# HaSai666/rec_pangu

Hardware: AMD Instinct MI355X
Metric: samples/sec DeepFM Criteo-shape bsz=65536/GPU (train step: fwd+bwd+dense Adam+zero_grad) (higher is better)
Workload: dtype f32

## Files before the change

rec_pangu_amd/csrc/mlp_tail.hip:

```cpp
#include "common.h"
#include "bfsplit.h"

#define MT_LD 72
#define MT_CT 68
#define MT_MAXL 3

struct TailFwdArgs {
    const float *W[MT_MAXL];
    const float *b[MT_MAXL];
    float *h[MT_MAXL];
    int64_t ldw[MT_MAXL];
};

__device__ __forceinline__ void mt_stage_w(const float *__restrict__ W, int64_t ldw, __bf16 (*Wt)[64][MT_LD]) {
    const int d = threadIdx.x >> 2, c = (threadIdx.x & 3) * 16;
    const float *src = W + (int64_t)d * ldw + c;
#pragma unroll
    for (int u = 0; u < 2; ++u) {
        const f32x4 v0 = *reinterpret_cast<const f32x4 *>(src + 8 * u), v1 = *reinterpret_cast<const f32x4 *>(src + 8 * u + 4);
        f32x8 v;
#pragma unroll
        for (int e = 0; e < 4; ++e) {
            v[e] = v0[e];
            v[4 + e] = v1[e];
        }
        bf16x8 pc[3];
        bf_split8<3>(v, pc);
#pragma unroll
        for (int q = 0; q < 3; ++q) *reinterpret_cast<bf16x8 *>(&Wt[q][d][c + 8 * u]) = pc[q];
    }
}

__device__ __forceinline__ void mt_stage_wt(const float *__restrict__ W, int64_t ldw, __bf16 (*Wt)[64][MT_LD]) {
    const int k = threadIdx.x >> 2, c = (threadIdx.x & 3) * 16;
    const float *src = W + (int64_t)k * ldw + c;
#pragma unroll
    for (int u = 0; u < 4; ++u) {
        const f32x4 v = *reinterpret_cast<const f32x4 *>(src + 4 * u);
#pragma unroll
        for (int e = 0; e < 4; ++e) {
            const float x = v[e];
            const __bf16 hi = (__bf16)x;
            const float r1 = x - (float)hi;
            const __bf16 mid = (__bf16)r1;
            const __bf16 lo = (__bf16)(r1 - (float)mid);
            const int n = c + 4 * u + e;
            Wt[0][n][k] = hi;
            Wt[1][n][k] = mid;
            Wt[2][n][k] = lo;
        }
    }
}

struct TailBce {
    const float *add[3];
    int n_add;
    const float *label;
    float p_eps;
    float *pred;
    float *partial;
};

template <int L, bool BCE>
__global__ __launch_bounds__(256, 2) void mlp_tail_fwd_kernel(const float *__restrict__ hin, int64_t ldin, TailFwdArgs a,
                                                              const float *__restrict__ wout, const float *__restrict__ bout,
                                                              float *__restrict__ logit, int64_t M, TailBce bc) {
    __shared__ __attribute__((aligned(16))) __bf16 Wt[3][64][MT_LD];
    __shared__ __attribute__((aligned(16))) float Ct[4][32][MT_CT];
    const int wv = threadIdx.x >> 6, l = threadIdx.x & 63, i = l & 31, h = l >> 5;
    const int64_t row = (int64_t)blockIdx.x * 128 + 32 * wv + i;
    const int64_t rowc = row < M ? row : M - 1;
    f32x8 av[4];
    {
        const float *src = hin + rowc * ldin + 8 * h;
#pragma unroll
        for (int ks = 0; ks < 4; ++ks) {
            const f32x4 v0 = *reinterpret_cast<const f32x4 *>(src + ks * 16), v1 = *reinterpret_cast<const f32x4 *>(src + ks * 16 + 4);
#pragma unroll
            for (int e = 0; e < 4; ++e) {
                av[ks][e] = v0[e];
                av[ks][4 + e] = v1[e];
            }
        }
    }
#pragma unroll
    for (int ly = 0; ly < L; ++ly) {
        if (ly > 0) __syncthreads();
        mt_stage_w(a.W[ly], a.ldw[ly], Wt);
        __syncthreads();
        f32x16 acc[2];
#pragma unroll
        for (int nt = 0; nt < 2; ++nt)
#pragma unroll
            for (int r = 0; r < 16; ++r) acc[nt][r] = 0.f;
#pragma unroll
        for (int ks = 0; ks < 4; ++ks) {
            bf16x8 af[3];
            bf_split8<3>(av[ks], af);
#pragma unroll
            for (int nt = 0; nt < 2; ++nt) {
                bf16x8 b[3];
#pragma unroll
                for (int q = 0; q < 3; ++q) b[q] = *reinterpret_cast<const bf16x8 *>(&Wt[q][nt * 32 + i][ks * 16 + 8 * h]);
#pragma unroll
                for (int pr = 0; pr < 6; ++pr)
                    acc[nt] = __builtin_amdgcn_mfma_f32_32x32x16_bf16(af[BfProd<6>::pa(pr)], b[BfProd<6>::pb(pr)], acc[nt], 0, 0, 0);
            }
        }
        float *hout = a.h[ly];
#pragma unroll
        for (int nt = 0; nt < 2; ++nt) {
            const int n = nt * 32 + i;
            const float bv = a.b[ly] != nullptr ? a.b[ly][n] : 0.f;
#pragma unroll
            for (int r = 0; r < 16; ++r) {
                const int rl = (r & 3) + 8 * (r >> 2) + 4 * h;
                const float v = fmaxf(acc[nt][r] + bv, 0.f);
                Ct[wv][rl][n] = v;
                const int64_t m = (int64_t)blockIdx.x * 128 + 32 * wv + rl;
                if (m < M) hout[m * 64 + n] = v;
            }
        }
        __syncthreads();
#pragma unroll
        for (int ks = 0; ks < 4; ++ks) {
            const f32x4 v0 = *reinterpret_cast<const f32x4 *>(&Ct[wv][i][ks * 16 + 8 * h]);
            const f32x4 v1 = *reinterpret_cast<const f32x4 *>(&Ct[wv][i][ks * 16 + 8 * h + 4]);
#pragma unroll
            for (int e = 0; e < 4; ++e) {
                av[ks][e] = v0[e];
                av[ks][4 + e] = v1[e];
            }
        }
    }
    float part = 0.f;
#pragma unroll
    for (int ks = 0; ks < 4; ++ks)
#pragma unroll
        for (int e = 0; e < 8; ++e) part = __builtin_fmaf(av[ks][e], wout[ks * 16 + 8 * h + e], part);
    part += __shfl_xor(part, 32, 64);
    const float lg = part + (bout != nullptr ? bout[0] : 0.f);
    if constexpr (!BCE) {
        if (h == 0 && row < M) logit[row] = lg;
    } else {
        __shared__ float lred[128];
        if (h == 0) {
            float term = 0.f;
            if (row < M) {
                float z = lg;
                if (bc.n_add > 0) {
                    z = bc.add[0][row];
                    for (int q = 1; q < bc.n_add; ++q) z += bc.add[q][row];
                    z += lg;
                }
                const float p = 1.f / (1.f + expf(-z));
                bc.pred[row] = p;
                const float pe = p + bc.p_eps, y = bc.label[row];
                const float lp = fmaxf(logf(pe), -100.f), l1p = fmaxf(log1pf(-pe), -100.f);
                term = -(y * lp + (1.f - y) * l1p);
            }
            lred[32 * wv + i] = term;
        }
        __syncthreads();
        if (threadIdx.x < 64) {
            float v = lred[threadIdx.x] + lred[threadIdx.x + 64];
#pragma unroll
            for (int o = 32; o >= 1; o >>= 1) v += __shfl_xor(v, o, 64);
            if (threadIdx.x == 0) bc.partial[blockIdx.x] = v;
        }
    }
}

extern "C" int rp_mlp_tail_fits(int n_hidden, int width, int64_t ldin) {
    return (n_hidden >= 1 && n_hidden <= MT_MAXL && width == 64 && ldin % 4 == 0) ? 1 : 0;
}

static int tail_fwd_launch(const float *hin, int64_t ldin, int n_hidden, const float *const *W_hidden, const int64_t *ldw,
                           const float *const *b_hidden, float *const *h_out, const float *w_out, const float *b_out,
                           float *logit, int64_t M, const TailBce *bce, rp_stream_t stream) {
    RP_REQUIRE(hin && W_hidden && ldw && b_hidden && h_out && w_out && (logit || bce), "mlp_tail_fwd: null pointer");
    if (!rp_mlp_tail_fits(n_hidden, 64, ldin) || !rp_aligned16(hin))
        return rp_fail(RP_ERR_UNSUPPORTED, "mlp_tail_fwd: 1..3 hidden layers of width 64, 16-byte aligned rows");
    if (M == 0) return RP_OK;
    TailFwdArgs a;
    for (int l = 0; l < MT_MAXL; ++l) {
        a.W[l] = nullptr;
        a.b[l] = nullptr;
        a.h[l] = nullptr;
        a.ldw[l] = 0;
    }
    for (int l = 0; l < n_hidden; ++l) {
        RP_REQUIRE(W_hidden[l] && h_out[l] && ldw[l] >= 64 && ldw[l] % 4 == 0 && rp_aligned16(W_hidden[l]),
                   "mlp_tail_fwd: layer %d invalid", l);
        a.W[l] = W_hidden[l];
        a.b[l] = b_hidden[l];
        a.h[l] = h_out[l];
        a.ldw[l] = ldw[l];
    }
    const dim3 grid((unsigned)rp_cdiv(M, 128));
    hipStream_t s = (hipStream_t)stream;
    TailBce bc{};
    if (bce != nullptr) bc = *bce;
#define TAIL_FWD(LL, BB) hipLaunchKernelGGL((mlp_tail_fwd_kernel<LL, BB>), grid, dim3(256), 0, s, hin, ldin, a, w_out, b_out, logit, M, bc)
    if (bce == nullptr) {
        if (n_hidden == 1) TAIL_FWD(1, false);
        else if (n_hidden == 2) TAIL_FWD(2, false);
        else TAIL_FWD(3, false);
    } else {
        if (n_hidden == 1) TAIL_FWD(1, true);
        else if (n_hidden == 2) TAIL_FWD(2, true);
        else TAIL_FWD(3, true);
    }
#undef TAIL_FWD
    RP_LAUNCH_CHECK("mlp_tail_fwd");
    return RP_OK;
}

extern "C" int rp_mlp_tail_fwd(const float *hin, int64_t ldin, int n_hidden, const float *const *W_hidden, const int64_t *ldw,
                               const float *const *b_hidden, float *const *h_out, const float *w_out, const float *b_out,
                               float *logit, int64_t M, rp_stream_t stream) {
    RP_REQUIRE(logit != nullptr, "mlp_tail_fwd: null pointer");
    return tail_fwd_launch(hin, ldin, n_hidden, W_hidden, ldw, b_hidden, h_out, w_out, b_out, logit, M, nullptr, stream);
}

extern "C" int rp_mlp_tail_loss_partials(int64_t M) { return (int)rp_cdiv(M > 0 ? M : 1, 128); }
// ... 7 lines not shown
    TailBce bc{};
    for (int q = 0; q < n_addends; ++q) {
        RP_REQUIRE(addends[q] != nullptr, "mlp_tail_fwd_bce: null addend %d", q);
        bc.add[q] = addends[q];
    }
    bc.n_add = n_addends;
    bc.label = label;
    bc.p_eps = p_eps;
    bc.pred = pred;
    bc.partial = partial;
    return tail_fwd_launch(hin, ldin, n_hidden, W_hidden, ldw, b_hidden, h_out, w_out, b_out, nullptr, M, &bc, stream);
}

struct TailBwdArgs {
    const float *W[MT_MAXL];
    const float *act[MT_MAXL + 1];
    int64_t ldw[MT_MAXL];
    int64_t ldact0;
};

struct TailDz {
    const float *pred, *label, *gloss;
    float p_eps, scale;
    float *dz_out;
};

template <int L>
__global__ __launch_bounds__(256, 2) void mlp_tail_bwd_kernel(const float *__restrict__ dz, TailBwdArgs a,
                                                              const float *__restrict__ wout, float *__restrict__ dhin,
                                                              int64_t lddh, float *__restrict__ P, int64_t M, int nwg, TailDz tz) {
    __shared__ __attribute__((aligned(16))) float T0[4][32][MT_CT];
    __shared__ __attribute__((aligned(16))) float T1[4][32][MT_CT];
    __shared__ float dzs[128];
    const int wv = threadIdx.x >> 6, l = threadIdx.x & 63, i = l & 31, h = l >> 5;
    const int64_t row0 = (int64_t)blockIdx.x * 128;
    const int64_t row = row0 + 32 * wv + i;
    const bool rok = row < M;
    const int64_t rowc = rok ? row : M - 1;
    const int mt = wv & 1, ntw = wv >> 1;
    float (*T0f)[MT_CT] = reinterpret_cast<float (*)[MT_CT]>(&T0[0][0][0]);
    float (*T1f)[MT_CT] = reinterpret_cast<float (*)[MT_CT]>(&T1[0][0][0]);
    float *Pg = P + (int64_t)blockIdx.x * ((int64_t)L * 64 * 64 + (int64_t)L * 64 + 64 + 1);
    float dzr = 0.f;
    if (tz.pred == nullptr) {
        dzr = rok ? dz[row] : 0.f;
    } else if (rok) {
        const float g = tz.gloss[0] * tz.scale;
        const float p = tz.pred[row], y = tz.label[row], pe = p + tz.p_eps;
        dzr = (pe - y) / fmaxf((1.f - pe) * pe, 1e-12f) * g;
        dzr *= p * (1.f - p);
        if (h == 0 && tz.dz_out != nullptr) tz.dz_out[row] = dzr;
    }
    if (h == 0) dzs[32 * wv + i] = dzr;
    f32x8 dp[4];
    {
        const float *src = a.act[L] + rowc * 64 + 8 * h;
#pragma unroll
        for (int ks = 0; ks < 4; ++ks) {
            const f32x4 v0 = *reinterpret_cast<const f32x4 *>(src + ks * 16), v1 = *reinterpret_cast<const f32x4 *>(src + ks * 16 + 4);
#pragma unroll
            for (int e = 0; e < 8; ++e) {
                const float av = e < 4 ? v0[e] : v1[e - 4];
                dp[ks][e] = av > 0.f ? dzr * wout[ks * 16 + 8 * h + e] : 0.f;
                T1[wv][i][ks * 16 + 8 * h + e] = rok ? dzr * av : 0.f;
            }
        }
    }
    __syncthreads();
    if (threadIdx.x < 64) {
        float s = 0.f;
        for (int r = 0; r < 128; ++r) s += T1f[r][threadIdx.x];
        Pg[(int64_t)L * 64 * 64 + (int64_t)L * 64 + threadIdx.x] = s;
    } else if (threadIdx.x == 64) {
        float s = 0.f;
        for (int r = 0; r < 128; ++r) s += dzs[r];
        Pg[(int64_t)L * 64 * 64 + (int64_t)L * 64 + 64] = s;
    }
#pragma unroll
    for (int ly = L; ly >= 1; --ly) {
        __syncthreads();
#pragma unroll
        for (int ks = 0; ks < 4; ++ks)
#pragma unroll
            for (int e = 0; e < 8; ++e) T0[wv][i][ks * 16 + 8 * h + e] = dp[ks][e];
        {
            const float *src = (ly - 1 == 0 ? a.act[0] + rowc * a.ldact0 : a.act[ly - 1] + rowc * 64) + 8 * h;
#pragma unroll
            for (int ks = 0; ks < 4; ++ks) {
                const f32x4 v0 = *reinterpret_cast<const f32x4 *>(src + ks * 16), v1 = *reinterpret_cast<const f32x4 *>(src + ks * 16 + 4);
                *reinterpret_cast<f32x4 *>(&T1[wv][i][ks * 16 + 8 * h]) = rok ? v0 : f32x4{0.f, 0.f, 0.f, 0.f};
                *reinterpret_cast<f32x4 *>(&T1[wv][i][ks * 16 + 8 * h + 4]) = rok ? v1 : f32x4{0.f, 0.f, 0.f, 0.f};
            }
        }
        bf16x8 wf[2][4][3];
        {
            const float *Wl = a.W[ly - 1];
            const int64_t ldw = a.ldw[ly - 1];
#pragma unroll
            for (int nt = 0; nt < 2; ++nt)
#pragma unroll
                for (int ks = 0; ks < 4; ++ks) {
                    f32x8 v;
#pragma unroll
                    for (int e = 0; e < 8; ++e) v[e] = Wl[(int64_t)(ks * 16 + 8 * h + e) * ldw + nt * 32 + i];
                    bf_split8<3>(v, wf[nt][ks]);
                }
        }
        __syncthreads();
        f32x16 wacc;
#pragma unroll
        for (int r = 0; r < 16; ++r) wacc[r] = 0.f;
        float bsum = 0.f;
#pragma unroll
        for (int ks = 0; ks < 8; ++ks) {
            f32x8 va, vb;
#pragma unroll
            for (int e = 0; e < 8; ++e) {
                va[e] = T0f[ks * 16 + 8 * h + e][mt * 32 + i];
                vb[e] = T1f[ks * 16 + 8 * h + e][ntw * 32 + i];
            }
            bsum += ((va[0] + va[1]) + (va[2] + va[3])) + ((va[4] + va[5]) + (va[6] + va[7]));
            bf16x8 pa_[3], pb_[3];
            bf_split8<3>(va, pa_);
            bf_split8<3>(vb, pb_);
#pragma unroll
            for (int pr = 0; pr < 6; ++pr)
                wacc = __builtin_amdgcn_mfma_f32_32x32x16_bf16(pa_[BfProd<6>::pa(pr)], pb_[BfProd<6>::pb(pr)], wacc, 0, 0, 0);
        }
        {
            float *Pw = Pg + (int64_t)(ly - 1) * 64 * 64;
#pragma unroll
            for (int r = 0; r < 16; ++r) Pw[(mt * 32 + (r & 3) + 8 * (r >> 2) + 4 * h) * 64 + ntw * 32 + i] = wacc[r];
            bsum += __shfl_xor(bsum, 32, 64);
            if (ntw == 0 && h == 0) Pg[(int64_t)L * 64 * 64 + (int64_t)(ly - 1) * 64 + mt * 32 + i] = bsum;
        }
        f32x16 acc[2];
#pragma unroll
        for (int nt = 0; nt < 2; ++nt)
#pragma unroll
            for (int r = 0; r < 16; ++r) acc[nt][r] = 0.f;
#pragma unroll
        for (int ks = 0; ks < 4; ++ks) {
            bf16x8 af[3];
            bf_split8<3>(dp[ks], af);
#pragma unroll
            for (int nt = 0; nt < 2; ++nt) {
#pragma unroll
                for (int pr = 0; pr < 6; ++pr)
                    acc[nt] = __builtin_amdgcn_mfma_f32_32x32x16_bf16(af[BfProd<6>::pa(pr)], wf[nt][ks][BfProd<6>::pb(pr)], acc[nt], 0, 0, 0);
            }
        }
        __syncthreads();
#pragma unroll
        for (int nt = 0; nt < 2; ++nt) {
            const int n = nt * 32 + i;
#pragma unroll
            for (int r = 0; r < 16; ++r) {
                const int rl = (r & 3) + 8 * (r >> 2) + 4 * h;
                const float v = T1[wv][rl][n] > 0.f ? acc[nt][r] : 0.f;
                if (ly - 1 == 0) {
                    const int64_t m = row0 + 32 * wv + rl;
                    if (m < M) dhin[m * lddh + n] = v;
                } else {
                    T0[wv][rl][n] = v;
                }
            }
        }
        if (ly - 1 > 0) {
            __syncthreads();
#pragma unroll
            for (int ks = 0; ks < 4; ++ks) {
                const f32x4 v0 = *reinterpret_cast<const f32x4 *>(&T0[wv][i][ks * 16 + 8 * h]);
                const f32x4 v1 = *reinterpret_cast<const f32x4 *>(&T0[wv][i][ks * 16 + 8 * h + 4]);
#pragma unroll
                for (int e = 0; e < 4; ++e) {
                    dp[ks][e] = v0[e];
                    dp[ks][4 + e] = v1[e];
                }
            }
        }
    }
}

__global__ __launch_bounds__(256) void mlp_tail_reduce_kernel(const float *__restrict__ P, int nwg, int64_t per, float *__restrict__ out) {
    __shared__ float red[16][17];
    const int c = threadIdx.x & 15, q = threadIdx.x >> 4;
    const int64_t e = (int64_t)blockIdx.x * 16 + c;
    float s = 0.f;
    if (e < per)
        for (int g = q; g < nwg; g += 16) s += P[(int64_t)g * per + e];
    red[q][c] = s;
    __syncthreads();
    if (q != 0 || e >= per) return;
#pragma unroll
    for (int j = 1; j < 16; ++j) s += red[j][c];
    out[e] = s;
}

extern "C" int rp_mlp_tail_bwd_workspace_bytes(int64_t M, int n_hidden, size_t *bytes) {
    RP_REQUIRE(bytes && M >= 0 && n_hidden >= 1 && n_hidden <= MT_MAXL, "mlp_tail_bwd_workspace_bytes: bad argument");
    const int64_t per = (int64_t)n_hidden * 64 * 64 + (int64_t)n_hidden * 64 + 64 + 1;
    *bytes = (size_t)(rp_cdiv(M > 0 ? M : 1, 128) * per) * sizeof(float) + 256;
// ... 81 lines not shown
```

rec_pangu_amd/csrc/embed_tiny.hip:

```cpp
#include "common.h"
#include "bfsplit.h"

#define ET_MAXF 16
#define ET_ROWS 224
#define ET_COLS 160
#define ET_LD 72
#define ET_CHUNK 64
#define ET_NOROW 254
#define ET_NOSMP 255

struct TinyTables {
    int n, total;
    int field[ET_MAXF];
    int base[ET_MAXF];
    int rows[ET_MAXF];
    int acc0[ET_MAXF];
};

__device__ __forceinline__ void tiny_split3(float v, __bf16 *p0, __bf16 *p1, __bf16 *p2) {
    uint32_t u = __float_as_uint(v);
    *reinterpret_cast<uint16_t *>(p0) = (uint16_t)(u >> 16);
    v -= __uint_as_float(u & 0xFFFF0000u);
    u = __float_as_uint(v);
    *reinterpret_cast<uint16_t *>(p1) = (uint16_t)(u >> 16);
    v -= __uint_as_float(u & 0xFFFF0000u);
    u = __float_as_uint(v);
    *reinterpret_cast<uint16_t *>(p2) = (uint16_t)(u >> 16);
}

__global__ __launch_bounds__(256, 2) void embed_grad_tiny_partial_kernel(
    const int32_t *__restrict__ keys, int64_t B, TinyTables tt, const float *__restrict__ dh, int64_t lddh,
    const float *__restrict__ sum_in, const float *__restrict__ gfm, int64_t per_blk, float *__restrict__ partial) {
    __shared__ __attribute__((aligned(16))) __bf16 Zt[3][ET_COLS][ET_LD];
    __shared__ __attribute__((aligned(8))) uint8_t rid[ET_MAXF][ET_CHUNK];
    __shared__ uint8_t rfld[ET_ROWS], rloc[ET_ROWS];
    const int t = threadIdx.x, wv = t >> 6, l = t & 63, i = l & 31, h = l >> 5;
    for (int m = t; m < ET_ROWS; m += 256) {
        int slot = 0, loc = ET_NOROW;
        for (int j = 0; j < tt.n; ++j)
            if (m >= tt.acc0[j] && m < tt.acc0[j] + tt.rows[j]) {
                slot = j;
                loc = m - tt.acc0[j];
            }
        rfld[m] = (uint8_t)slot;
        rloc[m] = (uint8_t)loc;
    }
    for (int e = t; e < 3 * (ET_COLS - 130) * ET_LD; e += 256) {
        const int p = e / ((ET_COLS - 130) * ET_LD), rest = e - p * ((ET_COLS - 130) * ET_LD);
        Zt[p][130 + rest / ET_LD][rest % ET_LD] = (__bf16)0.f;
    }
    f32x16 acc[5];
#pragma unroll
    for (int nt = 0; nt < 5; ++nt)
#pragma unroll
        for (int r = 0; r < 16; ++r) acc[nt][r] = 0.f;
    const int64_t s_begin = (int64_t)blockIdx.x * per_blk;
    const int64_t s_end = s_begin + per_blk < B ? s_begin + per_blk : B;
    __syncthreads();
    const int mt = 4 * (int)blockIdx.y + wv;
    const bool mok = mt < ET_ROWS / 32;
    const int fl0 = mok ? rfld[32 * mt + i] : 0, lc0 = mok ? rloc[32 * mt + i] : ET_NOROW;
    const int s = t >> 2, q = t & 3;
    f32x4 vd[4], vs[4];
    float g = 0.f, okf = 0.f;
    int rloc0 = ET_NOSMP, rloc1 = ET_NOSMP;
    auto fetch = [&](int64_t c0) {
        const int64_t b = c0 + s;
        const bool ok = b < s_end;
        const int64_t bc = ok ? b : s_end - 1;
        okf = ok ? 1.f : 0.f;
        g = (gfm != nullptr) ? gfm[bc] * okf : 0.f;
#pragma unroll
        for (int e = 0; e < 4; ++e) vd[e] = *reinterpret_cast<const f32x4 *>(dh + bc * lddh + 16 * q + 4 * e);
        if (sum_in != nullptr) {
#pragma unroll
            for (int e = 0; e < 4; ++e) vs[e] = *reinterpret_cast<const f32x4 *>(sum_in + bc * 64 + 16 * q + 4 * e);
        }
        rloc0 = rloc1 = ET_NOSMP;
        {
            const int idx = t, j = idx >> 6, ss = idx & 63;
            if (idx < tt.n * ET_CHUNK && c0 + ss < s_end) rloc0 = keys[(int64_t)tt.field[j] * B + c0 + ss] - tt.base[j];
        }
        {
            const int idx = t + 256, j = idx >> 6, ss = idx & 63;
            if (idx < tt.n * ET_CHUNK && c0 + ss < s_end) rloc1 = keys[(int64_t)tt.field[j] * B + c0 + ss] - tt.base[j];
        }
    };
    fetch(s_begin);
    for (int64_t c0 = s_begin; c0 < s_end; c0 += ET_CHUNK) {
        {
#pragma unroll
            for (int e = 0; e < 16; ++e) {
                const int col = 16 * q + e;
                tiny_split3(vd[e >> 2][e & 3] * okf, &Zt[0][col][s], &Zt[1][col][s], &Zt[2][col][s]);
                const float uval = (sum_in != nullptr) ? g * vs[e >> 2][e & 3] : 0.f;
                tiny_split3(uval, &Zt[0][64 + col][s], &Zt[1][64 + col][s], &Zt[2][64 + col][s]);
            }
            if (q == 0) tiny_split3(g, &Zt[0][128][s], &Zt[1][128][s], &Zt[2][128][s]);
            if (q == 1) tiny_split3(okf, &Zt[0][129][s], &Zt[1][129][s], &Zt[2][129][s]);
            if (t < tt.n * ET_CHUNK) rid[t >> 6][t & 63] = (uint8_t)rloc0;
            if (t + 256 < tt.n * ET_CHUNK) rid[(t + 256) >> 6][t & 63] = (uint8_t)rloc1;
            for (int idx = t + 512; idx < tt.n * ET_CHUNK; idx += 256) {
                const int j = idx >> 6, ss = idx & 63;
                int loc = ET_NOSMP;
                if (c0 + ss < s_end) loc = keys[(int64_t)tt.field[j] * B + c0 + ss] - tt.base[j];
                rid[j][ss] = (uint8_t)loc;
            }
        }
        if (c0 + ET_CHUNK < s_end) fetch(c0 + ET_CHUNK);
        __syncthreads();
#pragma unroll
        for (int ks = 0; ks < 4; ++ks) {
            const uint64_t r8 = *reinterpret_cast<const uint64_t *>(&rid[fl0][16 * ks + 8 * h]);
            u32x4 aw;
#pragma unroll
            for (int j = 0; j < 4; ++j) {
                const uint32_t e0 = (uint32_t)((r8 >> (16 * j)) & 0xFF), e1 = (uint32_t)((r8 >> (16 * j + 8)) & 0xFF);
                aw[j] = (e0 == (uint32_t)lc0 ? 0x00003F80u : 0u) | (e1 == (uint32_t)lc0 ? 0x3F800000u : 0u);
            }
            const bf16x8 a = __builtin_bit_cast(bf16x8, aw);
            if (mok) {
#pragma unroll
                for (int nt = 0; nt < 5; ++nt)
#pragma unroll
                    for (int p = 2; p >= 0; --p) {
                        const bf16x8 bq = *reinterpret_cast<const bf16x8 *>(&Zt[p][32 * nt + i][16 * ks + 8 * h]);
                        acc[nt] = __builtin_amdgcn_mfma_f32_32x32x16_bf16(a, bq, acc[nt], 0, 0, 0);
                    }
            }
        }
        __syncthreads();
    }
    float *P = partial + (int64_t)blockIdx.x * ET_ROWS * ET_COLS;
    if (mok) {
#pragma unroll
        for (int nt = 0; nt < 5; ++nt)
#pragma unroll
            for (int r = 0; r < 16; ++r)
                P[(int64_t)(32 * mt + (r & 3) + 8 * (r >> 2) + 4 * h) * ET_COLS + 32 * nt + i] = acc[nt][r];
    }
}

#define ET_FIN_PARTS 4
__global__ __launch_bounds__(ET_COLS * ET_FIN_PARTS) void embed_grad_tiny_finish_kernel(
    const float *__restrict__ partial, int nblk, TinyTables tt, const float *__restrict__ wt, int64_t ldwt,
    const float *__restrict__ arena, float *__restrict__ G, int accumulate, int has_fm, float *__restrict__ hs_out) {
    __shared__ float Sp[ET_FIN_PARTS][ET_COLS];
    __shared__ float S[ET_COLS];
    const int m = blockIdx.x, c = threadIdx.x % ET_COLS, part = threadIdx.x / ET_COLS;
    int slot = 0;
    for (int j = 0; j < tt.n; ++j)
        if (m >= tt.acc0[j] && m < tt.acc0[j] + tt.rows[j]) slot = j;
    const int64_t arow = (int64_t)tt.base[slot] + (m - tt.acc0[slot]);
    {
        const int per = (nblk + ET_FIN_PARTS - 1) / ET_FIN_PARTS;
        const int b0 = part * per, b1 = (b0 + per < nblk) ? b0 + per : nblk;
        float s = 0.f;
#pragma unroll 8
        for (int b = b0; b < b1; ++b) s += partial[((int64_t)b * ET_ROWS + m) * ET_COLS + c];
        Sp[part][c] = s;
    }
// ... 54 lines not shown
                                  int64_t ldwt, const float *gfm, const float *sum_in, const float *arena,
                                  float *grad_arena, int accumulate, float *dw, int64_t lddw, void *workspace,
                                  size_t workspace_bytes, rp_stream_t stream) {
    RP_REQUIRE(keys && tiny_field && tiny_base && tiny_rows && dh && wt && grad_arena && workspace, "embed_grad_tiny: null pointer");
    RP_REQUIRE(n_tiny >= 1 && n_tiny <= ET_MAXF, "embed_grad_tiny: %d tables (1..%d)", n_tiny, ET_MAXF);
    RP_REQUIRE(B >= 1 && B < INT32_MAX, "embed_grad_tiny: bad B");
    RP_REQUIRE(gfm == nullptr || arena != nullptr, "embed_grad_tiny: the FM term needs the arena");
    RP_REQUIRE(lddh % 4 == 0 && ldwt >= 64 && rp_aligned16(dh) && (sum_in == nullptr || rp_aligned16(sum_in)),
               "embed_grad_tiny: dh / sum_in rows must be 16-byte aligned");
    TinyTables tt;
    tt.n = n_tiny;
    int total = 0;
    for (int j = 0; j < ET_MAXF; ++j) {
        tt.field[j] = tt.base[j] = tt.rows[j] = tt.acc0[j] = 0;
        if (j >= n_tiny) continue;
        RP_REQUIRE(tiny_rows[j] >= 1 && tiny_rows[j] <= ET_NOROW, "embed_grad_tiny: table %d has %d rows (1..%d)", j, tiny_rows[j],
                   ET_NOROW);
        RP_REQUIRE(tiny_base[j] >= 0 && tiny_base[j] < INT32_MAX && tiny_field[j] >= 0, "embed_grad_tiny: bad table %d", j);
        tt.field[j] = tiny_field[j];
        tt.base[j] = (int)tiny_base[j];
        tt.rows[j] = tiny_rows[j];
        tt.acc0[j] = total;
        total += tiny_rows[j];
    }
    RP_REQUIRE(total <= ET_ROWS, "embed_grad_tiny: %d rows together (<= %d)", total, ET_ROWS);
    tt.total = total;
    const int64_t per = tiny_per_block(B);
    const int64_t nblk = rp_cdiv(B, per);
    size_t need = 0;
    rp_embed_grad_tiny_workspace_bytes(B, &need);
    RP_REQUIRE(workspace_bytes >= need, "embed_grad_tiny: workspace %zu < %zu bytes", workspace_bytes, need);
    float *partial = reinterpret_cast<float *>((reinterpret_cast<uintptr_t>(workspace) + 255) & ~(uintptr_t)255);
    hipStream_t s = (hipStream_t)stream;
    hipLaunchKernelGGL(embed_grad_tiny_partial_kernel, dim3((unsigned)nblk, 2), dim3(256), 0, s, keys, B, tt, dh, lddh, sum_in, gfm, per,
                       partial);
    RP_LAUNCH_CHECK("embed_grad_tiny (partial sums)");
    RP_REQUIRE(dw == nullptr || arena != nullptr, "embed_grad_tiny: the weight gradient needs the arena");
    float *hs = dw ? partial + (size_t)nblk * ET_ROWS * ET_COLS : nullptr;
    hipLaunchKernelGGL(embed_grad_tiny_finish_kernel, dim3((unsigned)total), dim3(ET_COLS * ET_FIN_PARTS), 0, s, partial, (int)nblk, tt, wt, ldwt, arena,
                       grad_arena, accumulate, gfm != nullptr ? 1 : 0, hs);
    RP_LAUNCH_CHECK("embed_grad_tiny (finish)");
    if (dw != nullptr) {
        for (int j = 0; j < n_tiny; ++j)
            RP_REQUIRE(lddw >= ((int64_t)tt.field[j] + 1) * 64, "embed_grad_tiny: dw rows shorter than field %d's columns", tt.field[j]);
        hipLaunchKernelGGL(embed_grad_tiny_dw_kernel, dim3((unsigned)n_tiny, 16), dim3(256), 0, s, hs, tt, arena, dw, lddw);
        RP_LAUNCH_CHECK("embed_grad_tiny (weight gradient)");
    }
    return RP_OK;
}
```

Measured before the change: 86.94 million.

## Prefetch weights and activations across layers in fused MLP tail kernels

The forward kernel now loads the next layer's weights into registers while the current layer computes. It writes hidden activations as coalesced 16-byte rows from the shared tile instead of scattered scalar stores, and it preloads biases, the output weight, labels and addends. Two block-wide barriers become wave-level syncs. The backward kernel prefetches the next layer's activations and transposed weights, stages W^T through shared memory (aliased onto T0) instead of uncoalesced per-lane global gathers, and vectorizes its tile writes. The cost is extra register pressure and an extra pair of barriers per backward layer.

After: 85.96 million. 0.989x the previous value.

```diff
diff --git a/profiles/microbench/mlp_tail.py b/profiles/microbench/mlp_tail.py
--- /dev/null
+++ b/profiles/microbench/mlp_tail.py
@@ -0,0 +1,77 @@
+import ctypes as C
+import json
+import sys
+import torch
+sys.path.insert(0, '.')
+from bench import HBM_COPY_GBS
+from rec_pangu_amd import hip
+
+args = [a for a in sys.argv[1:] if not a.startswith('--')]
+if '--lib' in sys.argv:
+    hip.LIB_PATH = sys.argv[sys.argv.index('--lib') + 1]
+    args.remove(hip.LIB_PATH)
+M = int(args[0]) if len(args) > 0 else 65536
+L = int(args[1]) if len(args) > 1 else 2
+reps = int(args[2]) if len(args) > 2 else 200
+lib = hip.lib()
+dev = 'cuda'
+g = torch.Generator(device=dev).manual_seed(0)
+rnd = lambda *s: torch.randn(*s, device=dev, generator=g)
+hin = rnd(M, 64).relu()
+Ws = [rnd(64, 64) / 8 for _ in range(L)]
+bs = [rnd(64) * 0.1 for _ in range(L)]
+w_out, b_out = rnd(1, 64) / 8, rnd(1)
+fm = rnd(M)
+label = (torch.rand(M, device=dev, generator=g) < 0.3).float()
+gloss = torch.tensor(1.0, device=dev)
+hs = [torch.empty(M, 64, device=dev) for _ in range(L)]
+pred = torch.empty(M, device=dev)
+n_part = lib.rp_mlp_tail_loss_partials(M)
+partial = torch.empty(n_part, device=dev)
+dhin = torch.empty(M, 64, device=dev)
+dz_out = torch.empty(M, device=dev)
+per = L * 4096 + L * 64 + 65
+grads = torch.empty(per, device=dev)
+nbytes = C.c_size_t(0)
+hip._check(lib.rp_mlp_tail_bwd_workspace_bytes(M, L, C.byref(nbytes)), "workspace")
+ws = torch.empty(nbytes.value, dtype=torch.uint8, device=dev)
+Wp, ldw = hip._ptr_array(Ws), hip._i64_array([64] * L)
+acts = hip._ptr_array([hin] + hs)
+
+
+def fwd():
+    hip._check(lib.rp_mlp_tail_fwd_bce(hin.data_ptr(), 64, L, Wp, ldw, hip._opt_ptr_array(bs), hip._ptr_array(hs), w_out.data_ptr(),
+                                       b_out.data_ptr(), hip._ptr_array([fm]), 1, label.data_ptr(), 0.0, pred.data_ptr(),
+                                       partial.data_ptr(), M, hip._stream()), "rp_mlp_tail_fwd_bce")
+
+
+def bwd():
+    hip._check(lib.rp_mlp_tail_bwd_bce(pred.data_ptr(), label.data_ptr(), gloss.data_ptr(), 0.0, 1.0, dz_out.data_ptr(), L, Wp, ldw,
+                                       acts, 64, w_out.data_ptr(), dhin.data_ptr(), 64, grads.data_ptr(), M, ws.data_ptr(),
+                                       nbytes.value, 1, hip._stream()), "rp_mlp_tail_bwd_bce")
+
+
+def time_us(fn):
+    for _ in range(20):
+        fn()
+    e0, e1 = torch.cuda.Event(enable_timing=True), torch.cuda.Event(enable_timing=True)
+    torch.cuda.synchronize()
+    e0.record()
+    for _ in range(reps):
+        fn()
+    e1.record()
+    torch.cuda.synchronize()
+    return e0.elapsed_time(e1) * 1e3 / reps
+
+
+nwg = (M + 127) // 128
+moved = {
+    "fwd": 4 * (M * 64 * (L + 1) + 3 * M + n_part) + 4 * L * 4160,
+    "bwd": 4 * (M * 64 * (L + 2) + 3 * M + nwg * per) + 4 * L * 4096,
+}
+for name, fn in (("fwd", fwd), ("bwd", bwd)):
+    us = time_us(fn)
+    gbs = moved[name] / us * 1e-3
+    print(json.dumps({"launch": f"mlp_tail_{name}_kernel<{L}>", "M": M, "lib": hip.LIB_PATH.split('/')[-2:], "alone_us": round(us, 2),
+                      "mbytes": round(moved[name] / 1e6, 2), "gb_per_s": round(gbs, 1),
+                      "frac_of_copy_ceiling": round(gbs / HBM_COPY_GBS, 3), "us_at_copy_ceiling": round(moved[name] / HBM_COPY_GBS * 1e-3, 2)}))
diff --git a/rec_pangu_amd/csrc/mlp_tail.hip b/rec_pangu_amd/csrc/mlp_tail.hip
--- a/rec_pangu_amd/csrc/mlp_tail.hip
+++ b/rec_pangu_amd/csrc/mlp_tail.hip
@@ -12,17 +12,23 @@
     int64_t ldw[MT_MAXL];
 };
 
-__device__ __forceinline__ void mt_stage_w(const float *__restrict__ W, int64_t ldw, __bf16 (*Wt)[64][MT_LD]) {
+
+__device__ __forceinline__ void mt_load_w(const float *__restrict__ W, int64_t ldw, f32x4 (&v)[4]) {
     const int d = threadIdx.x >> 2, c = (threadIdx.x & 3) * 16;
     const float *src = W + (int64_t)d * ldw + c;
 #pragma unroll
+    for (int u = 0; u < 4; ++u) v[u] = *reinterpret_cast<const f32x4 *>(src + 4 * u);
+}
+
+__device__ __forceinline__ void mt_store_w(const f32x4 (&r)[4], __bf16 (*Wt)[64][MT_LD]) {
+    const int d = threadIdx.x >> 2, c = (threadIdx.x & 3) * 16;
+#pragma unroll
     for (int u = 0; u < 2; ++u) {
-        const f32x4 v0 = *reinterpret_cast<const f32x4 *>(src + 8 * u), v1 = *reinterpret_cast<const f32x4 *>(src + 8 * u + 4);
         f32x8 v;
 #pragma unroll
         for (int e = 0; e < 4; ++e) {
-            v[e] = v0[e];
-            v[4 + e] = v1[e];
+            v[e] = r[2 * u][e];
+            v[4 + e] = r[2 * u + 1][e];
         }
         bf16x8 pc[3];
         bf_split8<3>(v, pc);
@@ -31,25 +37,31 @@
     }
 }
 
-__device__ __forceinline__ void mt_stage_wt(const float *__restrict__ W, int64_t ldw, __bf16 (*Wt)[64][MT_LD]) {
-    const int k = threadIdx.x >> 2, c = (threadIdx.x & 3) * 16;
-    const float *src = W + (int64_t)k * ldw + c;
-#pragma unroll
-    for (int u = 0; u < 4; ++u) {
-        const f32x4 v = *reinterpret_cast<const f32x4 *>(src + 4 * u);
-#pragma unroll
-        for (int e = 0; e < 4; ++e) {
-            const float x = v[e];
-            const __bf16 hi = (__bf16)x;
-            const float r1 = x - (float)hi;
-            const __bf16 mid = (__bf16)r1;
-            const __bf16 lo = (__bf16)(r1 - (float)mid);
-            const int n = c + 4 * u + e;
-            Wt[0][n][k] = hi;
-            Wt[1][n][k] = mid;
-            Wt[2][n][k] = lo;
-        }
-    }
+__device__ __forceinline__ void mt_load_wt(const float *__restrict__ W, int64_t ldw, float (&v)[16]) {
+    const int n = threadIdx.x & 63, kg = threadIdx.x >> 6;
+    const float *src = W + (int64_t)(16 * kg) * ldw + n;
+#pragma unroll
+    for (int e = 0; e < 16; ++e) v[e] = src[(int64_t)e * ldw];
+}
+
+__device__ __forceinline__ void mt_store_wt(const float (&r)[16], __bf16 (*Wt)[64][MT_LD]) {
+    const int n = threadIdx.x & 63, kg = threadIdx.x >> 6;
+#pragma unroll
+    for (int u = 0; u < 2; ++u) {
+        f32x8 v;
+#pragma unroll
+        for (int e = 0; e < 8; ++e) v[e] = r[8 * u + e];
+        bf16x8 pc[3];
+        bf_split8<3>(v, pc);
+#pragma unroll
+        for (int q = 0; q < 3; ++q) *reinterpret_cast<bf16x8 *>(&Wt[q][n][16 * kg + 8 * u]) = pc[q];
+    }
+}
+
+__device__ __forceinline__ void mt_wave_sync() {
+    __builtin_amdgcn_fence(__ATOMIC_RELEASE, "wavefront");
+    __builtin_amdgcn_wave_barrier();
+    __builtin_amdgcn_fence(__ATOMIC_ACQUIRE, "wavefront");
 }
 
 struct TailBce {
@@ -67,9 +79,12 @@
                                                               float *__restrict__ logit, int64_t M, TailBce bc) {
     __shared__ __attribute__((aligned(16))) __bf16 Wt[3][64][MT_LD];
     __shared__ __attribute__((aligned(16))) float Ct[4][32][MT_CT];
+    __shared__ __attribute__((aligned(16))) float wos[64];
     const int wv = threadIdx.x >> 6, l = threadIdx.x & 63, i = l & 31, h = l >> 5;
     const int64_t row = (int64_t)blockIdx.x * 128 + 32 * wv + i;
     const int64_t rowc = row < M ? row : M - 1;
+    f32x4 wr[4];
+    mt_load_w(a.W[0], a.ldw[0], wr);
     f32x8 av[4];
     {
         const float *src = hin + rowc * ldin + 8 * h;
@@ -83,10 +98,37 @@
             }
         }
     }
+    float bv[L][2];
+#pragma unroll
+    for (int ly = 0; ly < L; ++ly)
+#pragma unroll
+        for (int nt = 0; nt < 2; ++nt) bv[ly][nt] = a.b[ly] != nullptr ? a.b[ly][nt * 32 + i] : 0.f;
+    if (threadIdx.x < 64) wos[threadIdx.x] = wout[threadIdx.x];
+    const float bo = bout != nullptr ? bout[0] : 0.f;
+    float yl = 0.f, ad[3] = {0.f, 0.f, 0.f};
+    if constexpr (BCE) {
+        if (h == 0 && row < M) {
+            yl = bc.label[row];
+#pragma unroll
+            for (int q = 0; q < 3; ++q)
+                if (q < bc.n_add) ad[q] = bc.add[q][row];
+        }
+    }
+    auto store_rows = [&](float *hout) {
+        const int rs = l >> 4, cs = (l & 15) * 4;
+#pragma unroll
+        for (int j = 0; j < 8; ++j) {
+            const f32x4 v = *reinterpret_cast<const f32x4 *>(&Ct[wv][rs + 4 * j][cs]);
+            const int64_t m = (int64_t)blockIdx.x * 128 + 32 * wv + rs + 4 * j;
+            if (m < M) *reinterpret_cast<f32x4 *>(hout + m * 64 + cs) = v;
+        }
+    };
 #pragma unroll
     for (int ly = 0; ly < L; ++ly) {
         if (ly > 0) __syncthreads();
-        mt_stage_w(a.W[ly], a.ldw[ly], Wt);
+        mt_store_w(wr, Wt);
+        if (ly > 0) store_rows(a.h[ly - 1]);
+        if (ly + 1 < L) mt_load_w(a.W[ly + 1], a.ldw[ly + 1], wr);
         __syncthreads();
         f32x16 acc[2];
 #pragma unroll
@@ -107,21 +149,16 @@
                     acc[nt] = __builtin_amdgcn_mfma_f32_32x32x16_bf16(af[BfProd<6>::pa(pr)], b[BfProd<6>::pb(pr)], acc[nt], 0, 0, 0);
             }
         }
-        float *hout = a.h[ly];
 #pragma unroll
         for (int nt = 0; nt < 2; ++nt) {
             const int n = nt * 32 + i;
-            const float bv = a.b[ly] != nullptr ? a.b[ly][n] : 0.f;
 #pragma unroll
             for (int r = 0; r < 16; ++r) {
                 const int rl = (r & 3) + 8 * (r >> 2) + 4 * h;
-                const float v = fmaxf(acc[nt][r] + bv, 0.f);
-                Ct[wv][rl][n] = v;
-                const int64_t m = (int64_t)blockIdx.x * 128 + 32 * wv + rl;
-                if (m < M) hout[m * 64 + n] = v;
-            }
-        }
-        __syncthreads();
+                Ct[wv][rl][n] = fmaxf(acc[nt][r] + bv[ly][nt], 0.f);
+            }
+        }
+        mt_wave_sync();
 #pragma unroll
         for (int ks = 0; ks < 4; ++ks) {
             const f32x4 v0 = *reinterpret_cast<const f32x4 *>(&Ct[wv][i][ks * 16 + 8 * h]);
@@ -132,14 +169,18 @@
                 av[ks][4 + e] = v1[e];
             }
         }
+        if (ly + 1 == L) store_rows(a.h[ly]);
+        mt_wave_sync();
     }
     float part = 0.f;
 #pragma unroll
-    for (int ks = 0; ks < 4; ++ks)
-#pragma unroll
-        for (int e = 0; e < 8; ++e) part = __builtin_fmaf(av[ks][e], wout[ks * 16 + 8 * h + e], part);
+    for (int ks = 0; ks < 4; ++ks) {
+        const f32x4 w0 = *reinterpret_cast<const f32x4 *>(&wos[ks * 16 + 8 * h]), w1 = *reinterpret_cast<const f32x4 *>(&wos[ks * 16 + 8 * h + 4]);
+#pragma unroll
+        for (int e = 0; e < 8; ++e) part = __builtin_fmaf(av[ks][e], e < 4 ? w0[e] : w1[e - 4], part);
+    }
     part += __shfl_xor(part, 32, 64);
-    const float lg = part + (bout != nullptr ? bout[0] : 0.f);
+    const float lg = part + bo;
     if constexpr (!BCE) {
         if (h == 0 && row < M) logit[row] = lg;
     } else {
@@ -149,13 +190,15 @@
             if (row < M) {
                 float z = lg;
                 if (bc.n_add > 0) {
-                    z = bc.add[0][row];
-                    for (int q = 1; q < bc.n_add; ++q) z += bc.add[q][row];
+                    z = ad[0];
+#pragma unroll
+                    for (int q = 1; q < 3; ++q)
+                        if (q < bc.n_add) z += ad[q];
                     z += lg;
                 }
                 const float p = 1.f / (1.f + expf(-z));
                 bc.pred[row] = p;
-                const float pe = p + bc.p_eps, y = bc.label[row];
+                const float pe = p + bc.p_eps, y = yl;
                 const float lp = fmaxf(logf(pe), -100.f), l1p = fmaxf(log1pf(-pe), -100.f);
                 term = -(y * lp + (1.f - y) * l1p);
             }
@@ -190,7 +233,7 @@
         a.ldw[l] = 0;
     }
     for (int l = 0; l < n_hidden; ++l) {
-        RP_REQUIRE(W_hidden[l] && h_out[l] && ldw[l] >= 64 && ldw[l] % 4 == 0 && rp_aligned16(W_hidden[l]),
+        RP_REQUIRE(W_hidden[l] && h_out[l] && ldw[l] >= 64 && ldw[l] % 4 == 0 && rp_aligned16(W_hidden[l]) && rp_aligned16(h_out[l]),
                    "mlp_tail_fwd: layer %d invalid", l);
         a.W[l] = W_hidden[l];
         a.b[l] = b_hidden[l];
@@ -264,6 +307,8 @@
     __shared__ __attribute__((aligned(16))) float T0[4][32][MT_CT];
     __shared__ __attribute__((aligned(16))) float T1[4][32][MT_CT];
     __shared__ float dzs[128];
+    static_assert(sizeof(T0) >= 3 * 64 * MT_LD * sizeof(__bf16), "the W^T pieces share the dpre tile");
+    __bf16 (*Wt)[64][MT_LD] = reinterpret_cast<__bf16 (*)[64][MT_LD]>(&T0[0][0][0]);
     const int wv = threadIdx.x >> 6, l = threadIdx.x & 63, i = l & 31, h = l >> 5;
     const int64_t row0 = (int64_t)blockIdx.x * 128;
     const int64_t row = row0 + 32 * wv + i;
@@ -273,6 +318,26 @@
     float (*T0f)[MT_CT] = reinterpret_cast<float (*)[MT_CT]>(&T0[0][0][0]);
     float (*T1f)[MT_CT] = reinterpret_cast<float (*)[MT_CT]>(&T1[0][0][0]);
     float *Pg = P + (int64_t)blockIdx.x * ((int64_t)L * 64 * 64 + (int64_t)L * 64 + 64 + 1);
+    f32x4 aL[8], an[8];
+    float wr[2][16];
+    {
+        const float *src = a.act[L] + rowc * 64 + 8 * h;
+#pragma unroll
+        for (int ks = 0; ks < 4; ++ks) {
+            aL[2 * ks] = *reinterpret_cast<const f32x4 *>(src + ks * 16);
+            aL[2 * ks + 1] = *reinterpret_cast<const f32x4 *>(src + ks * 16 + 4);
+        }
+    }
+    auto load_act = [&](int ly) {
+        const float *src = (ly == 0 ? a.act[0] + rowc * a.ldact0 : a.act[ly] + rowc * 64) + 8 * h;
+#pragma unroll
+        for (int ks = 0; ks < 4; ++ks) {
+            an[2 * ks] = *reinterpret_cast<const f32x4 *>(src + ks * 16);
+            an[2 * ks + 1] = *reinterpret_cast<const f32x4 *>(src + ks * 16 + 4);
+        }
+    };
+    load_act(L - 1);
+    mt_load_wt(a.W[L - 1], a.ldw[L - 1], wr[(L - 1) & 1]);
     float dzr = 0.f;
     if (tz.pred == nullptr) {
         dzr = rok ? dz[row] : 0.f;
@@ -285,58 +350,49 @@
     }
     if (h == 0) dzs[32 * wv + i] = dzr;
     f32x8 dp[4];
-    {
-        const float *src = a.act[L] + rowc * 64 + 8 * h;
-#pragma unroll
-        for (int ks = 0; ks < 4; ++ks) {
-            const f32x4 v0 = *reinterpret_cast<const f32x4 *>(src + ks * 16), v1 = *reinterpret_cast<const f32x4 *>(src + ks * 16 + 4);
-#pragma unroll
-            for (int e = 0; e < 8; ++e) {
-                const float av = e < 4 ? v0[e] : v1[e - 4];
-                dp[ks][e] = av > 0.f ? dzr * wout[ks * 16 + 8 * h + e] : 0.f;
-                T1[wv][i][ks * 16 + 8 * h + e] = rok ? dzr * av : 0.f;
-            }
-        }
+    const float wol = wout[l];
+#pragma unroll
+    for (int ks = 0; ks < 4; ++ks) {
+        f32x4 p0, p1;
+        float dw[8];
+#pragma unroll
+        for (int e = 0; e < 8; ++e) dw[e] = dzr * __shfl(wol, ks * 16 + 8 * h + e, 64);
+#pragma unroll
+        for (int e = 0; e < 8; ++e) {
+            const float av = e < 4 ? aL[2 * ks][e] : aL[2 * ks + 1][e - 4];
+            dp[ks][e] = av > 0.f ? dw[e] : 0.f;
+            const float t = rok ? dzr * av : 0.f;
+            if (e < 4) p0[e] = t;
+            else p1[e - 4] = t;
+        }
+        *reinterpret_cast<f32x4 *>(&T1[wv][i][ks * 16 + 8 * h]) = p0;
+        *reinterpret_cast<f32x4 *>(&T1[wv][i][ks * 16 + 8 * h + 4]) = p1;
+        *reinterpret_cast<f32x4 *>(&T0[wv][i][ks * 16 + 8 * h]) = f32x4{dp[ks][0], dp[ks][1], dp[ks][2], dp[ks][3]};
+        *reinterpret_cast<f32x4 *>(&T0[wv][i][ks * 16 + 8 * h + 4]) = f32x4{dp[ks][4], dp[ks][5], dp[ks][6], dp[ks][7]};
     }
     __syncthreads();
     if (threadIdx.x < 64) {
         float s = 0.f;
+#pragma unroll 32
         for (int r = 0; r < 128; ++r) s += T1f[r][threadIdx.x];
         Pg[(int64_t)L * 64 * 64 + (int64_t)L * 64 + threadIdx.x] = s;
     } else if (threadIdx.x == 64) {
         float s = 0.f;
+#pragma unroll 32
         for (int r = 0; r < 128; ++r) s += dzs[r];
         Pg[(int64_t)L * 64 * 64 + (int64_t)L * 64 + 64] = s;
     }
+    __syncthreads();
 #pragma unroll
     for (int ly = L; ly >= 1; --ly) {
-        __syncthreads();
-#pragma unroll
-        for (int ks = 0; ks < 4; ++ks)
-#pragma unroll
-            for (int e = 0; e < 8; ++e) T0[wv][i][ks * 16 + 8 * h + e] = dp[ks][e];
-        {
-            const float *src = (ly - 1 == 0 ? a.act[0] + rowc * a.ldact0 : a.act[ly - 1] + rowc * 64) + 8 * h;
-#pragma unroll
-            for (int ks = 0; ks < 4; ++ks) {
-                const f32x4 v0 = *reinterpret_cast<const f32x4 *>(src + ks * 16), v1 = *reinterpret_cast<const f32x4 *>(src + ks * 16 + 4);
-                *reinterpret_cast<f32x4 *>(&T1[wv][i][ks * 16 + 8 * h]) = rok ? v0 : f32x4{0.f, 0.f, 0.f, 0.f};
-                *reinterpret_cast<f32x4 *>(&T1[wv][i][ks * 16 + 8 * h + 4]) = rok ? v1 : f32x4{0.f, 0.f, 0.f, 0.f};
-            }
-        }
-        bf16x8 wf[2][4][3];
-        {
-            const float *Wl = a.W[ly - 1];
-            const int64_t ldw = a.ldw[ly - 1];
-#pragma unroll
-            for (int nt = 0; nt < 2; ++nt)
-#pragma unroll
-                for (int ks = 0; ks < 4; ++ks) {
-                    f32x8 v;
-#pragma unroll
-                    for (int e = 0; e < 8; ++e) v[e] = Wl[(int64_t)(ks * 16 + 8 * h + e) * ldw + nt * 32 + i];
-                    bf_split8<3>(v, wf[nt][ks]);
-                }
+#pragma unroll
+        for (int ks = 0; ks < 4; ++ks) {
+            *reinterpret_cast<f32x4 *>(&T1[wv][i][ks * 16 + 8 * h]) = rok ? an[2 * ks] : f32x4{0.f, 0.f, 0.f, 0.f};
+            *reinterpret_cast<f32x4 *>(&T1[wv][i][ks * 16 + 8 * h + 4]) = rok ? an[2 * ks + 1] : f32x4{0.f, 0.f, 0.f, 0.f};
+        }
+        if (ly >= 2) {
+            load_act(ly - 2);
+            mt_load_wt(a.W[ly - 2], a.ldw[ly - 2], wr[(ly - 2) & 1]);
         }
         __syncthreads();
         f32x16 wacc;
@@ -366,6 +422,9 @@
             bsum += __shfl_xor(bsum, 32, 64);
             if (ntw == 0 && h == 0) Pg[(int64_t)L * 64 * 64 + (int64_t)(ly - 1) * 64 + mt * 32 + i] = bsum;
         }
+        __syncthreads();
+        mt_store_wt(wr[(ly - 1) & 1], Wt);
+        __syncthreads();
         f32x16 acc[2];
 #pragma unroll
         for (int nt = 0; nt < 2; ++nt)
@@ -377,9 +436,12 @@
             bf_split8<3>(dp[ks], af);
 #pragma unroll
             for (int nt = 0; nt < 2; ++nt) {
+                bf16x8 b[3];
+#pragma unroll
+                for (int q = 0; q < 3; ++q) b[q] = *reinterpret_cast<const bf16x8 *>(&Wt[q][nt * 32 + i][ks * 16 + 8 * h]);
 #pragma unroll
                 for (int pr = 0; pr < 6; ++pr)
-                    acc[nt] = __builtin_amdgcn_mfma_f32_32x32x16_bf16(af[BfProd<6>::pa(pr)], wf[nt][ks][BfProd<6>::pb(pr)], acc[nt], 0, 0, 0);
+                    acc[nt] = __builtin_amdgcn_mfma_f32_32x32x16_bf16(af[BfProd<6>::pa(pr)], b[BfProd<6>::pb(pr)], acc[nt], 0, 0, 0);
             }
         }
         __syncthreads();
@@ -399,7 +461,7 @@
             }
         }
         if (ly - 1 > 0) {
-            __syncthreads();
+            mt_wave_sync();
 #pragma unroll
             for (int ks = 0; ks < 4; ++ks) {
                 const f32x4 v0 = *reinterpret_cast<const f32x4 *>(&T0[wv][i][ks * 16 + 8 * h]);
```

## Merge tiny-embedding grad grid halves into one 512-thread block with packed bf16 staging

Applied to the files above, without the earlier changes.

The partial-sum kernel now runs one 512-thread block per sample range instead of two 256-thread blocks (grid y=2). The old layout had both blocks stage the same chunk into shared memory; now the chunk is staged once and all seven row tiles read it. Staging is reorganised so each thread splits two samples at a time into packed bf16 pairs and writes 32-bit words, cutting LDS store count. Key loads are spread across waves, and the MFMA loop preloads all B operands ahead of a sched_barrier before issuing the 15 MFMAs. The tradeoff is fewer blocks in flight, so less occupancy across CUs, plus higher register pressure from holding the preloaded operands.

Result: no change. 84.79 million before, 85.01 million after (median of 2 runs) (+0.3%).

```diff
diff --git a/rec_pangu_amd/csrc/embed_tiny.hip b/rec_pangu_amd/csrc/embed_tiny.hip
--- a/rec_pangu_amd/csrc/embed_tiny.hip
+++ b/rec_pangu_amd/csrc/embed_tiny.hip
@@ -6,6 +6,7 @@
 #define ET_COLS 160
 #define ET_LD 72
 #define ET_CHUNK 64
+#define ET_THREADS 512
 #define ET_NOROW 254
 #define ET_NOSMP 255
 
@@ -17,25 +18,24 @@
     int acc0[ET_MAXF];
 };
 
-__device__ __forceinline__ void tiny_split3(float v, __bf16 *p0, __bf16 *p1, __bf16 *p2) {
-    uint32_t u = __float_as_uint(v);
-    *reinterpret_cast<uint16_t *>(p0) = (uint16_t)(u >> 16);
-    v -= __uint_as_float(u & 0xFFFF0000u);
-    u = __float_as_uint(v);
-    *reinterpret_cast<uint16_t *>(p1) = (uint16_t)(u >> 16);
-    v -= __uint_as_float(u & 0xFFFF0000u);
-    u = __float_as_uint(v);
-    *reinterpret_cast<uint16_t *>(p2) = (uint16_t)(u >> 16);
-}
-
-__global__ __launch_bounds__(256, 2) void embed_grad_tiny_partial_kernel(
+__device__ __forceinline__ void tiny_split3_pair(float va, float vb, uint32_t (&w)[3]) {
+#pragma unroll
+    for (int p = 0; p < 3; ++p) {
+        const uint32_t ua = __float_as_uint(va), ub = __float_as_uint(vb);
+        w[p] = (ua >> 16) | (ub & 0xFFFF0000u);
+        va -= __uint_as_float(ua & 0xFFFF0000u);
+        vb -= __uint_as_float(ub & 0xFFFF0000u);
+    }
+}
+
+__global__ __launch_bounds__(ET_THREADS) void embed_grad_tiny_partial_kernel(
     const int32_t *__restrict__ keys, int64_t B, TinyTables tt, const float *__restrict__ dh, int64_t lddh,
     const float *__restrict__ sum_in, const float *__restrict__ gfm, int64_t per_blk, float *__restrict__ partial) {
-    __shared__ __attribute__((aligned(16))) __bf16 Zt[3][ET_COLS][ET_LD];
+    __shared__ __attribute__((aligned(16))) uint32_t Zt[3][ET_COLS][ET_LD / 2];
     __shared__ __attribute__((aligned(8))) uint8_t rid[ET_MAXF][ET_CHUNK];
     __shared__ uint8_t rfld[ET_ROWS], rloc[ET_ROWS];
     const int t = threadIdx.x, wv = t >> 6, l = t & 63, i = l & 31, h = l >> 5;
-    for (int m = t; m < ET_ROWS; m += 256) {
+    for (int m = t; m < ET_ROWS; m += ET_THREADS) {
         int slot = 0, loc = ET_NOROW;
         for (int j = 0; j < tt.n; ++j)
             if (m >= tt.acc0[j] && m < tt.acc0[j] + tt.rows[j]) {
@@ -45,9 +45,9 @@
         rfld[m] = (uint8_t)slot;
         rloc[m] = (uint8_t)loc;
     }
-    for (int e = t; e < 3 * (ET_COLS - 130) * ET_LD; e += 256) {
-        const int p = e / ((ET_COLS - 130) * ET_LD), rest = e - p * ((ET_COLS - 130) * ET_LD);
-        Zt[p][130 + rest / ET_LD][rest % ET_LD] = (__bf16)0.f;
+    for (int e = t; e < 3 * (ET_COLS - 130) * (ET_LD / 2); e += ET_THREADS) {
+        const int p = e / ((ET_COLS - 130) * (ET_LD / 2)), rest = e - p * ((ET_COLS - 130) * (ET_LD / 2));
+        Zt[p][130 + rest / (ET_LD / 2)][rest % (ET_LD / 2)] = 0u;
     }
     f32x16 acc[5];
 #pragma unroll
@@ -57,76 +57,99 @@
     const int64_t s_begin = (int64_t)blockIdx.x * per_blk;
     const int64_t s_end = s_begin + per_blk < B ? s_begin + per_blk : B;
     __syncthreads();
-    const int mt = 4 * (int)blockIdx.y + wv;
+    const int mt = wv;
     const bool mok = mt < ET_ROWS / 32;
     const int fl0 = mok ? rfld[32 * mt + i] : 0, lc0 = mok ? rloc[32 * mt + i] : ET_NOROW;
-    const int s = t >> 2, q = t & 3;
-    f32x4 vd[4], vs[4];
-    float g = 0.f, okf = 0.f;
-    int rloc0 = ET_NOSMP, rloc1 = ET_NOSMP;
+    const int sp = i, cg = 2 * wv + h;
+    const bool is_s = cg >= 8;
+    const bool live = !is_s || sum_in != nullptr;
+    const float *src = (is_s && sum_in != nullptr) ? sum_in + 8 * (cg - 8) : dh + 8 * (cg & 7);
+    const int64_t ldsrc = (is_s && sum_in != nullptr) ? 64 : lddh;
+    const float *gsrc = gfm != nullptr ? gfm : dh;
+    int64_t koff[2];
+    int kbase[2];
+    bool kok[2];
+#pragma unroll
+    for (int e = 0; e < 2; ++e) {
+        const int j = wv + 8 * e;
+        int fld = 0, bs = 0;
+#pragma unroll
+        for (int jj = 0; jj < ET_MAXF; ++jj)
+            if (jj == j) {
+                fld = tt.field[jj];
+                bs = tt.base[jj];
+            }
+        kok[e] = j < tt.n;
+        koff[e] = kok[e] ? (int64_t)fld * B : 0;
+        kbase[e] = bs;
+    }
+    f32x4 va[2], vb[2];
+    float g0 = 0.f, g1 = 0.f;
+    int kraw[2] = {0, 0};
     auto fetch = [&](int64_t c0) {
-        const int64_t b = c0 + s;
-        const bool ok = b < s_end;
-        const int64_t bc = ok ? b : s_end - 1;
-        okf = ok ? 1.f : 0.f;
-        g = (gfm != nullptr) ? gfm[bc] * okf : 0.f;
-#pragma unroll
-        for (int e = 0; e < 4; ++e) vd[e] = *reinterpret_cast<const f32x4 *>(dh + bc * lddh + 16 * q + 4 * e);
-        if (sum_in != nullptr) {
-#pragma unroll
-            for (int e = 0; e < 4; ++e) vs[e] = *reinterpret_cast<const f32x4 *>(sum_in + bc * 64 + 16 * q + 4 * e);
-        }
-        rloc0 = rloc1 = ET_NOSMP;
-        {
-            const int idx = t, j = idx >> 6, ss = idx & 63;
-            if (idx < tt.n * ET_CHUNK && c0 + ss < s_end) rloc0 = keys[(int64_t)tt.field[j] * B + c0 + ss] - tt.base[j];
-        }
-        {
-            const int idx = t + 256, j = idx >> 6, ss = idx & 63;
-            if (idx < tt.n * ET_CHUNK && c0 + ss < s_end) rloc1 = keys[(int64_t)tt.field[j] * B + c0 + ss] - tt.base[j];
+        const int64_t ba = c0 + 2 * sp, bb = ba + 1, bs = c0 + l;
+        const int64_t bca = ba < s_end ? ba : s_end - 1, bcb = bb < s_end ? bb : s_end - 1, bcs = bs < s_end ? bs : s_end - 1;
+        g0 = gsrc[bca];
+        g1 = gsrc[bcb];
+#pragma unroll
+        for (int e = 0; e < 2; ++e) kraw[e] = keys[koff[e] + bcs];
+#pragma unroll
+        for (int e = 0; e < 2; ++e) {
+            va[e] = *reinterpret_cast<const f32x4 *>(src + bca * ldsrc + 4 * e);
+            vb[e] = *reinterpret_cast<const f32x4 *>(src + bcb * ldsrc + 4 * e);
         }
     };
     fetch(s_begin);
     for (int64_t c0 = s_begin; c0 < s_end; c0 += ET_CHUNK) {
         {
-#pragma unroll
-            for (int e = 0; e < 16; ++e) {
-                const int col = 16 * q + e;
-                tiny_split3(vd[e >> 2][e & 3] * okf, &Zt[0][col][s], &Zt[1][col][s], &Zt[2][col][s]);
-                const float uval = (sum_in != nullptr) ? g * vs[e >> 2][e & 3] : 0.f;
-                tiny_split3(uval, &Zt[0][64 + col][s], &Zt[1][64 + col][s], &Zt[2][64 + col][s]);
-            }
-            if (q == 0) tiny_split3(g, &Zt[0][128][s], &Zt[1][128][s], &Zt[2][128][s]);
-            if (q == 1) tiny_split3(okf, &Zt[0][129][s], &Zt[1][129][s], &Zt[2][129][s]);
-            if (t < tt.n * ET_CHUNK) rid[t >> 6][t & 63] = (uint8_t)rloc0;
-            if (t + 256 < tt.n * ET_CHUNK) rid[(t + 256) >> 6][t & 63] = (uint8_t)rloc1;
-            for (int idx = t + 512; idx < tt.n * ET_CHUNK; idx += 256) {
-                const int j = idx >> 6, ss = idx & 63;
-                int loc = ET_NOSMP;
-                if (c0 + ss < s_end) loc = keys[(int64_t)tt.field[j] * B + c0 + ss] - tt.base[j];
-                rid[j][ss] = (uint8_t)loc;
-            }
+            const float oka = c0 + 2 * sp < s_end ? 1.f : 0.f, okb = c0 + 2 * sp + 1 < s_end ? 1.f : 0.f;
+            const float ga = gfm != nullptr ? g0 * oka : 0.f, gb = gfm != nullptr ? g1 * okb : 0.f;
+            const float ma = is_s ? ga : oka, mb = is_s ? gb : okb;
+            uint32_t w[3];
+#pragma unroll
+            for (int e = 0; e < 8; ++e) {
+                const float xa = live ? va[e >> 2][e & 3] * ma : 0.f, xb = live ? vb[e >> 2][e & 3] * mb : 0.f;
+                tiny_split3_pair(xa, xb, w);
+#pragma unroll
+                for (int p = 0; p < 3; ++p) Zt[p][8 * cg + e][sp] = w[p];
+            }
+            if (t < 32) {
+                tiny_split3_pair(ga, gb, w);
+#pragma unroll
+                for (int p = 0; p < 3; ++p) Zt[p][128][sp] = w[p];
+            } else if (t < 64) {
+                tiny_split3_pair(oka, okb, w);
+#pragma unroll
+                for (int p = 0; p < 3; ++p) Zt[p][129][sp] = w[p];
+            }
+            const bool s_in = c0 + l < s_end;
+#pragma unroll
+            for (int e = 0; e < 2; ++e) rid[wv + 8 * e][l] = (uint8_t)((kok[e] && s_in) ? kraw[e] - kbase[e] : ET_NOSMP);
         }
         if (c0 + ET_CHUNK < s_end) fetch(c0 + ET_CHUNK);
         __syncthreads();
-#pragma unroll
-        for (int ks = 0; ks < 4; ++ks) {
-            const uint64_t r8 = *reinterpret_cast<const uint64_t *>(&rid[fl0][16 * ks + 8 * h]);
-            u32x4 aw;
-#pragma unroll
-            for (int j = 0; j < 4; ++j) {
-                const uint32_t e0 = (uint32_t)((r8 >> (16 * j)) & 0xFF), e1 = (uint32_t)((r8 >> (16 * j + 8)) & 0xFF);
-                aw[j] = (e0 == (uint32_t)lc0 ? 0x00003F80u : 0u) | (e1 == (uint32_t)lc0 ? 0x3F800000u : 0u);
-            }
-            const bf16x8 a = __builtin_bit_cast(bf16x8, aw);
-            if (mok) {
-#pragma unroll
-                for (int nt = 0; nt < 5; ++nt)
-#pragma unroll
-                    for (int p = 2; p >= 0; --p) {
-                        const bf16x8 bq = *reinterpret_cast<const bf16x8 *>(&Zt[p][32 * nt + i][16 * ks + 8 * h]);
-                        acc[nt] = __builtin_amdgcn_mfma_f32_32x32x16_bf16(a, bq, acc[nt], 0, 0, 0);
-                    }
+        if (mok) {
+#pragma unroll
+            for (int ks = 0; ks < 4; ++ks) {
+                bf16x8 bq[3][5];
+#pragma unroll
+                for (int p = 2; p >= 0; --p)
+#pragma unroll
+                    for (int nt = 0; nt < 5; ++nt)
+                        bq[p][nt] = *reinterpret_cast<const bf16x8 *>(&Zt[p][32 * nt + i][8 * ks + 4 * h]);
+                const uint64_t r8 = *reinterpret_cast<const uint64_t *>(&rid[fl0][16 * ks + 8 * h]);
+                u32x4 aw;
+#pragma unroll
+                for (int j = 0; j < 4; ++j) {
+                    const uint32_t e0 = (uint32_t)((r8 >> (16 * j)) & 0xFF), e1 = (uint32_t)((r8 >> (16 * j + 8)) & 0xFF);
+                    aw[j] = (e0 == (uint32_t)lc0 ? 0x00003F80u : 0u) | (e1 == (uint32_t)lc0 ? 0x3F800000u : 0u);
+                }
+                const bf16x8 a = __builtin_bit_cast(bf16x8, aw);
+                __builtin_amdgcn_sched_barrier(0);
+#pragma unroll
+                for (int p = 2; p >= 0; --p)
+#pragma unroll
+                    for (int nt = 0; nt < 5; ++nt) acc[nt] = __builtin_amdgcn_mfma_f32_32x32x16_bf16(a, bq[p][nt], acc[nt], 0, 0, 0);
             }
         }
         __syncthreads();
@@ -247,7 +270,7 @@
     RP_REQUIRE(workspace_bytes >= need, "embed_grad_tiny: workspace %zu < %zu bytes", workspace_bytes, need);
     float *partial = reinterpret_cast<float *>((reinterpret_cast<uintptr_t>(workspace) + 255) & ~(uintptr_t)255);
     hipStream_t s = (hipStream_t)stream;
-    hipLaunchKernelGGL(embed_grad_tiny_partial_kernel, dim3((unsigned)nblk, 2), dim3(256), 0, s, keys, B, tt, dh, lddh, sum_in, gfm, per,
+    hipLaunchKernelGGL(embed_grad_tiny_partial_kernel, dim3((unsigned)nblk), dim3(ET_THREADS), 0, s, keys, B, tt, dh, lddh, sum_in, gfm, per,
                        partial);
     RP_LAUNCH_CHECK("embed_grad_tiny (partial sums)");
     RP_REQUIRE(dw == nullptr || arena != nullptr, "embed_grad_tiny: the weight gradient needs the arena");
```
